# JasonTStanley/MultiDroneSim

Measured on AMD Instinct MI355X. Metric: drone-steps/sec (whole node) at N_envs×N_drones; achieved HBM GB/s vs roofline, higher is better.
Workload: dtype f32

## Files before the change

include/mds.h:

```cpp
#ifndef MDS_H
#define MDS_H

#include <stddef.h>
#include <stdint.h>

#ifdef __cplusplus
extern "C" {
#endif

#define MDS_VERSION 202
#define MDS_OBS_DIM 20
#define MDS_ACT_DIM 4
#define MDS_STATE_DIM 13
#define MDS_DES_DIM 11
#define MDS_LEM_DIM 7
#define MDS_GEO_AUX_DIM 13

typedef enum mds_status {
  MDS_OK = 0,
  MDS_EINVAL = -1,
  MDS_ENOMEM = -2,
  MDS_EHIP = -3,
  MDS_EALIGN = -4,
  MDS_ESTATE = -5,
// ... 50 lines not shown

int mds_set_origin(mds_handle* h, const double* origin_host, void* stream);

int mds_get_obs(mds_handle* h, void* obs_dev, void* stream);

int mds_step(mds_handle* h, const void* action_dev, void* obs_dev, void* stream);

int mds_set_wind(mds_handle* h, const double force_world[3]);

#define MDS_SEG_DIM 40
int mds_set_trajectory_segments(mds_handle* h, const double* segs_host, const int32_t* offsets_host,
                                const int32_t* compound_host, const double* anchor_host, int32_t total_segments, void* stream);
int mds_traj_eval(mds_handle* h, double t, void* des_dev, void* stream);

int mds_set_lemniscate(mds_handle* h, const double* params_host, void* stream);
int mds_set_geometric_gains(mds_handle* h, const mds_geometric_gains* gains);

int mds_step_geometric(mds_handle* h, double t, void* obs_dev, void* action_dev, void* stream);

int mds_rollout_geometric(mds_handle* h, double t0, int n_steps, void* obs_dev, int obs_every_step, void* stream);

int mds_rollout_step(mds_handle* h, const void* actions_dev, int n_action_sets, int first_step, int n_steps, void* obs_log_dev,
                     int log_slots, int episode_len, void* stream);
int mds_rollout_step_fused(mds_handle* h, const void* actions_dev, int n_action_sets, int first_step, int n_steps, void* obs_log_dev,
                           int log_slots, int episode_len, int steps_per_launch, void* stream);
int mds_reset_async(mds_handle* h, void* stream);

int mds_set_rollout_streams(mds_handle* h, int n_streams);
int mds_get_last_rollout_streams(const mds_handle* h);
int mds_rollout_streams_for(const mds_handle* h, int loop, int n_steps);
// ... 125 lines not shown
```

multidronesim_amd/_capi.py:

```python
from __future__ import annotations

import ctypes as C
import os

_HERE = os.path.dirname(os.path.abspath(__file__))
LIB_PATH = os.environ.get("MDS_LIB_PATH") or os.path.join(_HERE, "libmds.so")

MDS_OK = 0
MDS_F32, MDS_F64, MDS_F16, MDS_F32C = 0, 1, 2, 3
MDS_PHYSICS_DYN, MDS_PHYSICS_DYN_DRAG, MDS_PHYSICS_DYN_GND, MDS_PHYSICS_DYN_DW, MDS_PHYSICS_DYN_GND_DRAG_DW = 0, 1, 2, 3, 4
MDS_INTEGRATOR_EULER, MDS_INTEGRATOR_RK4 = 0, 1
MDS_CF2X, MDS_CF2P = 0, 1
OBS_DIM, ACT_DIM, STATE_DIM, DES_DIM, LEM_DIM, GEO_AUX_DIM, SEG_DIM = 20, 4, 13, 11, 7, 13, 40


class MdsConfig(C.Structure):
    _fields_ = [("num_envs", C.c_int32), ("num_drones", C.c_int32), ("dtype", C.c_int32), ("physics", C.c_int32),
                ("integrator", C.c_int32), ("drone_model", C.c_int32), ("pyb_freq", C.c_int32),
                ("ctrl_freq", C.c_int32), ("device", C.c_int32), ("track_last_rpm", C.c_int32),
                ("M", C.c_double), ("L", C.c_double), ("KF", C.c_double), ("KM", C.c_double), ("J", C.c_double * 3),
                ("G", C.c_double), ("thrust2weight", C.c_double), ("drag_coeff", C.c_double * 3)]


class MdsGeometricGains(C.Structure):
# ... 26 lines not shown
    "mds_last_error": (C.c_char_p, []),
    "mds_default_config": (C.c_int, [C.c_int, C.POINTER(MdsConfig)]),
    "mds_default_geometric_gains": (C.c_int, [C.POINTER(MdsGeometricGains)]),
    "mds_create": (C.c_int, [C.POINTER(MdsConfig), C.POINTER(_P)]),
    "mds_destroy": (C.c_int, [_P]),
    "mds_get_derived": (C.c_int, [_P, _PD]),
    "mds_reset": (C.c_int, [_P, _PD, _PD, _P]),
    "mds_state_ptrs": (C.c_int, [_P, C.POINTER(C.c_void_p), C.POINTER(C.c_size_t), C.POINTER(C.c_void_p)]),
    "mds_get_state": (C.c_int, [_P, _PD, _P]),
    "mds_set_state": (C.c_int, [_P, _PD, _P]),
    "mds_set_origin": (C.c_int, [_P, _PD, _P]),
    "mds_get_obs": (C.c_int, [_P, _P, _P]),
    "mds_step": (C.c_int, [_P, _P, _P, _P]),
    "mds_set_wind": (C.c_int, [_P, _PD]),
    "mds_set_lemniscate": (C.c_int, [_P, _PD, _P]),
    "mds_set_trajectory_segments": (C.c_int, [_P, _PD, C.POINTER(C.c_int32), C.POINTER(C.c_int32), _PD, C.c_int32, _P]),
    "mds_traj_eval": (C.c_int, [_P, C.c_double, _P, _P]),
    "mds_set_geometric_gains": (C.c_int, [_P, C.POINTER(MdsGeometricGains)]),
    "mds_step_geometric": (C.c_int, [_P, C.c_double, _P, _P, _P]),
    "mds_rollout_geometric": (C.c_int, [_P, C.c_double, C.c_int, _P, C.c_int, _P]),
    "mds_set_rollout_streams": (C.c_int, [_P, C.c_int]),
    "mds_get_last_rollout_streams": (C.c_int, [_P]),
    "mds_rollout_streams_for": (C.c_int, [_P, C.c_int, C.c_int]),
    "mds_set_rollout_form": (C.c_int, [_P, C.c_int, C.c_int]),
    "mds_rollout_form_for": (C.c_int, [_P, C.c_int]),
    "mds_get_last_rollout_form": (C.c_int, [_P]),
    "mds_rollout_step": (C.c_int, [_P, _P, C.c_int, C.c_int, C.c_int, _P, C.c_int, C.c_int, _P]),
    "mds_rollout_step_fused": (C.c_int, [_P, _P, C.c_int, C.c_int, C.c_int, _P, C.c_int, C.c_int, C.c_int, _P]),
    "mds_reset_async": (C.c_int, [_P, _P]),
    "mds_rollout_geometric_fused": (C.c_int, [_P, C.c_double, C.c_int, _P, _P, _P]),
# ... 98 lines not shown
```

multidronesim_amd/csrc/mds_api.hip:

```cpp
#include <hip/hip_runtime.h>
#include <math.h>
#include <stdio.h>
#include <stdlib.h>
#include <string.h>

#include <new>
#include <type_traits>
#include <unordered_map>
#include <vector>

#include "../../include/mds.h"
#include "mds_consts.hpp"
#include "mds_kernels.hip"
#include "mds_traj_image.hpp"
#ifndef MDS_PART
#define MDS_PART 3
#endif
#if MDS_PART & 2
#include "mds_cbf_kernels.hip"
#include "mds_fedce_kernels.hip"
#include "mds_fedce_omega_kernels.hip"
#include "mds_care_kernels.hip"
#else
#include "mds_cbf.hpp"
// ... 69 lines not shown
struct mds_handle {
  mds_config cfg = {};
  mds_geometric_gains gains = {};
  double wind[3] = {0.0, 0.0, 0.0};
  int n = 0;
  size_t ld = 0;
  void* state = nullptr;
  void* state_lo = nullptr;
  void* origin = nullptr;
  void* last_rpm = nullptr;
  void* lem = nullptr;
  double* scratch = nullptr;
  double* init_pose = nullptr;
  bool has_traj = false;
  int traj_mode = 0;
  double* segs = nullptr;
  int nseg_total = 0;
  int* tinfo = nullptr;
  HostParams<float> p32 = {};
  HostParams<double> p64 = {};
  bool has_cbf = false;
  mds_cbf_params cbf = {};
  int* pair_ij = nullptr;
  void* obstacles = nullptr;
  int* cbf_order = nullptr;
  int* cbf_count = nullptr;
  int cbf_calls_half[2] = {-1, -1};
  int* cbf_cost = nullptr;
  int cbf_calls = -1;
  int rollout_streams = 0;
// ... 564 lines not shown
  if (!aligned16(action) || !aligned16(obs)) return fail(MDS_EALIGN, "mds_step: action_dev/obs_dev");
  hipStream_t st = (hipStream_t)stream;
  if (h->envfx) return step_env_plain(h, action, obs, st, 0);
  launch_step_plain(h, action, obs, st);
  MDS_HIP(hipGetLastError());
  return MDS_OK;
}

int mds_set_lemniscate(mds_handle* h, const double* params, void* stream) {
  MDS_DEV(h);
  if (!h || !params) return fail(MDS_EINVAL, "mds_set_lemniscate: null argument");
  hipStream_t st = (hipStream_t)stream;
  const int n = h->n;
  double* centres = new (std::nothrow) double[(size_t)n * 3];
  if (!centres) return fail(MDS_ENOMEM, "mds_set_lemniscate: host allocation");
  for (int i = 0; i < n; ++i)
    for (int k = 0; k < 3; ++k) centres[(size_t)3 * i + k] = params[(size_t)7 * i + 2 + k];
  int rc = mds_set_origin(h, centres, stream);
  delete[] centres;
  if (rc != MDS_OK) return rc;
  MDS_HIP(hipMemcpyAsync(h->scratch, params, (size_t)n * 7 * sizeof(double), hipMemcpyHostToDevice, st));
  with_dtype(h->cfg.dtype, [&](auto DT) {
    using T = typename decltype(DT)::T;
    k_set_planes<T><<<grid_for(n, 256), 256, 0, st>>>(n, h->ld, 7, h->scratch, (T*)h->lem);
  });
  MDS_HIP(hipGetLastError());
  MDS_HIP(hipStreamSynchronize(st));
  h->has_traj = true;
  h->traj_mode = 1;
  return MDS_OK;
}

int mds_set_trajectory_segments(mds_handle* h, const double* segs, const int32_t* offsets, const int32_t* compound,
                                const double* anchor, int32_t total, void* stream) {
  MDS_DEV(h);
  if (!h || !segs || !offsets || !compound || !anchor) return fail(MDS_EINVAL, "mds_set_trajectory_segments: null argument");
  const int n = h->n;
  std::vector<int> ti;
  std::vector<double> fm;
  int nu = 0;
  const char* why = "";
  const int brc = build_traj_image(segs, offsets, compound, n, total, fm, ti, nu, &why);
  if (brc != MDS_OK) return fail(brc, why);
  int rc = mds_set_origin(h, anchor, stream);
  if (rc != MDS_OK) return rc;
  hipError_t e = hipSuccess;
  if (h->segs) (void)hipFree(h->segs);
  h->segs = nullptr;
  h->nseg_total = 0;
  if (!h->tinfo) e = hipMalloc((void**)&h->tinfo, sizeof(int) * 3 * n);
  if (e == hipSuccess) e = hipMalloc((void**)&h->segs, sizeof(double) * fm.size());
  if (e == hipSuccess) e = hipMemcpy(h->segs, fm.data(), sizeof(double) * fm.size(), hipMemcpyHostToDevice);
  if (e == hipSuccess) e = hipMemcpy(h->tinfo, ti.data(), sizeof(int) * 3 * n, hipMemcpyHostToDevice);
  if (e != hipSuccess) return fail_hip(e, "mds_set_trajectory_segments");
  h->nseg_total = nu;
  h->has_traj = true;
  h->traj_mode = 2;
  return MDS_OK;
}

int mds_traj_eval(mds_handle* h, double t, void* des, void* stream) {
  MDS_DEV(h);
  if (!h || !des) return fail(MDS_EINVAL, "mds_traj_eval: null argument");
  if (h->traj_mode == 1) return mds_lemniscate_eval(h, t, des, stream);
  if (h->traj_mode != 2) return fail(MDS_ESTATE, "mds_traj_eval: no trajectories set");
  hipStream_t st = (hipStream_t)stream;
  with_dtype(h->cfg.dtype, [&](auto DT) {
    using S = typename decltype(DT)::S;
    k_traj_eval<S><<<grid_for(h->n, 256), 256, 0, st>>>(h->n, t, SegTable{h->segs, h->nseg_total}, h->tinfo, (S*)des);
  });
  MDS_HIP(hipGetLastError());
  return MDS_OK;
// ... 18 lines not shown
  const unsigned nbatch = nb ? nb : (unsigned)((h->n + kBlock - 1) / kBlock);
  const size_t pad = nb ? split_lds_pad(h, h->traj_mode == 2 || obs) : 0;
  const dim3 grid(nbatch);
  const bool rk4 = h->cfg.integrator == MDS_INTEGRATOR_RK4, drag = has_drag(h);
  if (h->traj_mode == 2) {
    with_flags([&](auto RK4, auto DRAG) {
      with_dtype(h->cfg.dtype, [&](auto DT) {
        using T = typename decltype(DT)::T; using S = typename decltype(DT)::S;
        k_step_traj<T, S, RK4(), DRAG(), DT.COMP><<<grid, kBlock, pad, st>>>(params<T>(h).c, h->n, h->ld, t, (S*)h->state, (const T*)h->origin,
                                                                             SegTable{h->segs, h->nseg_total}, h->tinfo, (T*)rpm_track(h), (S*)obs,
                                                                             (S*)act, (int)batch0, (S*)h->state_lo);
      });
    }, rk4, drag);
    return MDS_OK;
  }
  with_flags([&](auto HAS_OBS, auto HAS_ACT, auto RK4, auto DRAG) {
    with_dtype(h->cfg.dtype, [&](auto DT) {
      using T = typename decltype(DT)::T; using S = typename decltype(DT)::S;
      k_step_geometric<T, S, HAS_OBS(), HAS_ACT(), RK4(), DRAG(), DT.COMP><<<grid, kBlock, pad, st>>>(params<T>(h).c, h->n, h->ld, t, (S*)h->state,
                                                                                                      (const T*)h->lem, (T*)rpm_track(h), (S*)obs,
                                                                                                      (S*)act, (int)batch0, (S*)h->state_lo);
    });
  }, obs != nullptr, act != nullptr, rk4, drag);
  return MDS_OK;
}

int mds_step_geometric(mds_handle* h, double t, void* obs, void* act, void* stream) {
  MDS_DEV(h);
  if (!h) return fail(MDS_EINVAL, "mds_step_geometric: null handle");
  if (!h->has_traj) return fail(MDS_ESTATE, "mds_step_geometric: call mds_set_lemniscate first");
  if (!aligned16(obs) || !aligned16(act)) return fail(MDS_EALIGN, "mds_step_geometric: obs_dev/action_dev");
  if (h->envfx) return step_env_ctrl(h, 0, t, nullptr, 0.0, obs, act, (hipStream_t)stream);
  launch_step_geometric(h, t, obs, act, (hipStream_t)stream);
  MDS_HIP(hipGetLastError());
  return MDS_OK;
}

static void launch_rollout_kernel(mds_handle* h, int ctrl, double t0, int n_steps, void* obs_log, size_t log_stride, void* obs_last, hipStream_t st) {
// ... 1 lines not shown
  const double dt = 1.0 / h->cfg.ctrl_freq;
  const int omode = obs_log == nullptr ? kObsLast : log_stride == 0 ? kObsInPlace : kObsLog;
  auto launch = [&](auto DT, auto CTRL) {
    using T = typename decltype(DT)::T; using S = typename decltype(DT)::S;
    constexpr int COMP = DT.COMP ? 1 : 0;
    const void* gain = nullptr;
    if constexpr (CTRL() >= 1) gain = h->gain_dev[CTRL() - 1];
    with_flags([&](auto RK4, auto DRAG) {
      auto roll = [&](auto OBS) {
        if (h->traj_mode == 2) {
          if constexpr (CTRL() <= 1)
            k_rollout_traj<T, S, RK4(), DRAG(), CTRL(), COMP, OBS()><<<grid, kBlock, 0, st>>>(
                params<T>(h).c, gain, h->n, h->ld, t0, dt, n_steps, (S*)h->state, (const T*)h->origin, SegTable{h->segs, h->nseg_total}, h->tinfo,
                (T*)rpm_track(h), (S*)obs_log, log_stride, (S*)obs_last, (S*)h->state_lo);
        } else {
          k_rollout_geometric<T, S, RK4(), DRAG(), CTRL(), COMP, OBS()><<<grid, kBlock, 0, st>>>(
              params<T>(h).c, gain, h->n, h->ld, t0, dt, n_steps, (S*)h->state, (const T*)h->lem, (T*)rpm_track(h), (S*)obs_log, log_stride,
              (S*)obs_last, (T*)h->ll, (const S*)obs_last, (S*)h->state_lo);
        }
      };
      constexpr bool kPerObs = sizeof(T) == 4 && !RK4() && !DRAG() && CTRL() == 0;
      if constexpr (kPerObs) with_int<kObsInPlace, kObsLog, kObsLast>(omode, roll);
      else roll(std::integral_constant<int, -1>{});
    }, h->cfg.integrator == MDS_INTEGRATOR_RK4, has_drag(h));
  };
  if (ctrl >= 2) with_int<2, 3>(ctrl, [&](auto CTRL) { with_dtype_no_half(h->cfg.dtype, [&](auto DT) { launch(DT, CTRL); }); });
  else with_int<1, 0>(ctrl, [&](auto CTRL) { with_dtype(h->cfg.dtype, [&](auto DT) { launch(DT, CTRL); }); });
}

int mds_rollout_geometric(mds_handle* h, double t0, int n_steps, void* obs, int obs_every_step, void* stream) {
  MDS_DEV(h);
  if (!h || n_steps < 0) return fail(MDS_EINVAL, "mds_rollout_geometric");
  if (!h->has_traj) return fail(MDS_ESTATE, "mds_rollout_geometric: call mds_set_lemniscate first");
// ... 1678 lines not shown
```

multidronesim_amd/csrc/mds_kernels.hip:

```cpp
#include <hip/hip_runtime.h>
#include <type_traits>

#include "mds_math.hpp"
#include "mds_traj.hpp"

namespace mds {

typedef _Float16 half_t;

constexpr int kBlock = 256;
constexpr int kWave = 64;
constexpr int kStepMinWaves = 4;

#if defined(__HIP_DEVICE_COMPILE__)
#define MDS_KEEP_V(x) asm volatile("" : "+v"(x))
#define MDS_KEEP_S(x) asm volatile("" : "+s"(x))
#else
#define MDS_KEEP_V(x) ((void)0)
#define MDS_KEEP_S(x) ((void)0)
#endif
#if defined(__HIP_DEVICE_COMPILE__) || defined(__HIPCC__)
#define MDS_CONST_AS __attribute__((address_space(4)))
#else
#define MDS_CONST_AS
// ... 421 lines not shown
  T a[4];
  load4<T, T>(lem + 4 * i, a);
  struct alignas(2 * sizeof(T)) V2 {
    T v[2];
  };
  const V2 c = *reinterpret_cast<const V2*>(lem + 4 * ld + 2 * i);
  in.P.a = a[0];
  in.P.omega = a[1];
  in.P.yaw_rate = a[2];
  in.P.phase_shift = a[3];
  in.P.cx = c.v[0];
  in.P.cy = c.v[1];
  in.P.cz = lem[6 * ld + i];
}

template <typename T, typename S, bool HAS_OBS, bool HAS_ACT, bool RK4, bool DRAG, bool COMP = false>
__device__ __forceinline__ void geo_process(const Consts<T>& c, const int n, const size_t ld, const double t, const int i,
                                            GeoIn<T>& in, S* __restrict__ state, T* __restrict__ last_rpm,
                                            S* __restrict__ obs, S* __restrict__ action_out, unsigned char* lds,
                                            S* __restrict__ state_lo = nullptr) {
  const bool valid = i < n;
  T o[kObsDim];
  if (valid) {
    State<T>& s = in.s;
    const LemniscateParams<T>& P = in.P;
    T prev[4] = {T(0), T(0), T(0), T(0)}, clipped[4], act[4];
    if (DRAG)
      for (int k = 0; k < 4; ++k) prev[k] = last_rpm[k * ld + i];
    {
      const Desired<T> des = lemniscate_local(P, t);
      const Frame<T> F = make_frame(s.q, s.w);
      T u[4];
      geometric_control<T>(c, s.p - des.p, F.R, s.v, F.av, des, u, nullptr);
      input_to_action(c, u, act);
      if (COMP) aviary_step_comp<T, RK4, DRAG>(c, s, in.r, act, prev, clipped);
      else aviary_step<T, RK4, DRAG>(c, s, F, act, prev, clipped);
    }
    if (DRAG || last_rpm)
      for (int k = 0; k < 4; ++k) last_rpm[k * ld + i] = clipped[k];
    if (HAS_ACT) store4<S, T>(action_out + (size_t)i * 4, act);
    if (HAS_OBS) pack_obs(s, V3<T>{P.cx, P.cy, P.cz}, clipped, o);
  }
  if (HAS_OBS) write_obs_rows<S, T>(lds, obs, n, i, valid, o);
  if (valid) {
    store_state<S, T>(state, ld, i, in.s);
    if (COMP) store_resid<S, T>(state_lo, ld, i, in.r);
  }
}

template <typename T, typename S, bool HAS_OBS, bool HAS_ACT, bool RK4, bool DRAG, bool COMP = false>
__global__ __launch_bounds__(kBlock, 1) void k_step_geometric(const Consts<T> c, const int n, const size_t ld, const double t,
                                                           S* __restrict__ state, const T* __restrict__ lem,
                                                           T* __restrict__ last_rpm, S* __restrict__ obs,
                                                           S* __restrict__ action_out, const int batch0,
                                                           S* __restrict__ state_lo = nullptr) {
  __shared__ __align__(16) unsigned char lds[HAS_OBS ? (kBlock * kObsDim * sizeof(S)) : 16];
  const int i = (batch0 + blockIdx.x) * kBlock + threadIdx.x;
  GeoIn<T> in;
  if (i < n) {
    load_geo_in<T, S>(state, lem, ld, i, in);
    if (COMP) load_resid<S, T>(state_lo, ld, i, in.r);
  }
  geo_process<T, S, HAS_OBS, HAS_ACT, RK4, DRAG, COMP>(c, n, ld, t, i, in, state, last_rpm, obs, action_out, lds, state_lo);
}

template <typename T, typename S, bool RK4, bool DRAG, bool COMP = false>
__global__ __launch_bounds__(kBlock) void k_step_traj(const Consts<T> c, const int n, const size_t ld, const double t,
                                                      S* __restrict__ state, const T* __restrict__ origin,
                                                      const SegTable segs, const int* __restrict__ tinfo,
                                                      T* __restrict__ last_rpm, S* __restrict__ obs, S* __restrict__ action_out,
                                                      const int batch0, S* __restrict__ state_lo = nullptr) {
  __shared__ __align__(16) unsigned char lds[kBlock * kObsDim * sizeof(S)];
  const int i = (batch0 + blockIdx.x) * kBlock + threadIdx.x;
  const bool valid = i < n;
  T o[kObsDim];
  State<T> s;
  Resid<T> r;
  if (valid) {
// ... 85 lines not shown

template <typename S>
__global__ void k_traj_eval(const int n, const double t, const SegTable segs, const int* __restrict__ tinfo,
                            S* __restrict__ des) {
  const int i = blockIdx.x * blockDim.x + threadIdx.x;
  if (i >= n) return;
  double d11[11];
  traj_eval(segs, traj_info(tinfo, i), t, d11);
  for (int k = 0; k < 11; ++k) des[(size_t)i * 11 + k] = (S)d11[k];
}

constexpr int kObsLast = 0, kObsInPlace = 1, kObsLog = 2;
template <typename T, bool RK4, bool DRAG, int CTRL, int COMP, int OBS> constexpr int rollout_min_waves() {
  return !(sizeof(T) == 4 && !RK4 && !DRAG && CTRL == 0 && COMP == 0) ? 1 : (OBS == kObsInPlace || OBS == kObsLog) ? 6 : OBS == kObsLast ? 5 : 1;
}
template <typename T, typename S, bool RK4, bool DRAG, int CTRL = 0, int COMP = -1, int OBS = -1>
__global__ __launch_bounds__(kBlock, (rollout_min_waves<T, RK4, DRAG, CTRL, COMP, OBS>())) void k_rollout_geometric(
    const Consts<T> c_arg, const void* __restrict__ Kp, const int n, const size_t ld, double t, const double ctrl_dt, const int n_steps,
    S* __restrict__ state, const T* __restrict__ lem, T* __restrict__ last_rpm, S* __restrict__ obs_log, const size_t log_stride,
    S* __restrict__ obs_last, T* __restrict__ ll = nullptr, const S* __restrict__ obs_prev = nullptr, S* __restrict__ state_lo = nullptr) {
  __shared__ __align__(16) unsigned char lds[kBlock * kObsDim * sizeof(S)];
  const bool comp = COMP < 0 ? state_lo != nullptr : COMP != 0;
  const int omode = OBS < 0 ? (obs_log == nullptr ? kObsLast : log_stride == 0 ? kObsInPlace : kObsLog) : OBS;
  constexpr bool kLean = !RK4 && COMP != 1;
  const int i = blockIdx.x * kBlock + threadIdx.x;
  const bool valid = i < n;
  if (n <= 0) return;
  const size_t il = (size_t)min(i, n - 1);
  GeoIn<T> in;
  resid_zero(in.r);
  if (comp) load_resid<S, T>(state_lo, ld, il, in.r);
  T prev[4] = {T(0), T(0), T(0), T(0)};
  T thr[4] = {T(0), T(0), T(0), T(0)};
  LowLevelState<T> L;
  L.last_omega = L.integral = {T(0), T(0), T(0)};
  load_geo_in<T, S>(state, lem, ld, il, in);
// ... 12 lines not shown
  for (int k = 0; k < n_steps; ++k) {
    T o[kObsDim];
    const bool last = k == n_steps - 1;
    const bool want = omode != kObsLast || (obs_last != nullptr && last);
#if defined(__HIP_DEVICE_COMPILE__)
    const Consts<T> MDS_CONST_AS* cp = (const Consts<T> MDS_CONST_AS*)__builtin_amdgcn_kernarg_segment_ptr();
    MDS_KEEP_S(cp);
    const Consts<T> c = kLean ? load_const(cp) : c_arg;
#else
    const Consts<T>& c = c_arg;
#endif
    T act[4], clipped[4];
    {
      if (kLean) {
        MDS_KEEP_V(in.P.a);
        MDS_KEEP_V(in.P.yaw_rate);
      }
      const Desired<T> des = lemniscate_local(in.P, t);
      T u[4];
      if (CTRL == 0) {
        if (!kCarry) {
          F = make_frame(in.s.q, in.s.w);
        } else if (kLean) {
          MDS_KEEP_V(F.r22m1);
          F.R.m[8] = T(1) + F.r22m1;
        }
        geometric_control<T>(c, in.s.p - des.p, F.R, in.s.v, F.av, des, u, nullptr);
      } else if (CTRL == 1) {
        lqr12_control<T>(c, *static_cast<const Lqr12Gain<T>*>(Kp), euler_from_quat(in.s.q), quat_rotate(in.s.q, in.s.w), in.s.v, in.s.p - des.p,
                         des.v, des.yaw, des.yaw_rate, u);
      } else if (CTRL == 2) {
        lqr_omega_control<T>(c, *static_cast<const LqrGain<T>*>(Kp), euler_from_quat(in.s.q), in.s.v, in.s.p, des.p, des.v, des.yaw, u);
      } else {
        lqr_yank_omega_control<T>(c, *static_cast<const LqrYoGain<T>*>(Kp), euler_from_quat(in.s.q), thr, in.s.v, in.s.p, des.p, des.v,
                                  des.yaw, u);
      }
      if (CTRL <= 1) input_to_action(c, u, act);
      else if (CTRL == 2) thrust_omega_control(c, (T)ctrl_dt, u, in.s.w, L, act);
      else yank_omega_control(c, (T)ctrl_dt, u, thr, in.s.w, L, act);
    }
    if (comp) aviary_step_comp<T, RK4, DRAG>(c, in.s, in.r, act, prev, clipped);
    else if (CTRL == 0) aviary_step<T, RK4, DRAG>(c, in.s, F, act, prev, clipped);
// ... 14 lines not shown
    if (omode == kObsInPlace) write_obs_rows<S, T, true, kLean>(lds, obs_log, n, i, valid, o, ro);
    else if (omode == kObsLog) write_obs_rows<S, T, false, kLean>(lds, obs_log + (size_t)k * log_stride, n, i, valid, o, ro);
    if (omode != kObsInPlace && obs_last != nullptr && last) write_obs_rows<S, T, false, kLean>(lds, obs_last, n, i, valid, o, ro);
    t = uniform_f64(t + ctrl_dt);
  }
  if (valid) {
    store_state<S, T>(state, ld, i, in.s);
    if (comp) store_resid<S, T>(state_lo, ld, i, in.r);
    if (DRAG && n_steps <= 0)
      for (int k = 0; k < 4; ++k) last_rpm[k * ld + i] = prev[k];
    if (CTRL >= 2) {
      ll[0 * ld + i] = L.last_omega.x; ll[1 * ld + i] = L.last_omega.y; ll[2 * ld + i] = L.last_omega.z;
      ll[3 * ld + i] = L.integral.x; ll[4 * ld + i] = L.integral.y; ll[5 * ld + i] = L.integral.z;
    }
  }
}

template <typename T, typename S, bool RK4, bool DRAG, int CTRL, int COMP = -1, int OBS = -1>
__global__ __launch_bounds__(kBlock) void k_rollout_traj(const Consts<T> c, const void* __restrict__ Kp, const int n, const size_t ld, double t,
                                                         const double ctrl_dt, const int n_steps, S* __restrict__ state,
                                                         const T* __restrict__ origin, const SegTable segs,
                                                         const int* __restrict__ tinfo, T* __restrict__ last_rpm,
                                                         S* __restrict__ obs_log, const size_t log_stride, S* __restrict__ obs_last,
                                                         S* __restrict__ state_lo = nullptr) {
  __shared__ __align__(16) unsigned char lds[kBlock * kObsDim * sizeof(S)];
  const bool comp = COMP < 0 ? state_lo != nullptr : COMP != 0;
  const int omode = OBS < 0 ? (obs_log == nullptr ? kObsLast : log_stride == 0 ? kObsInPlace : kObsLog) : OBS;
  const int i = blockIdx.x * kBlock + threadIdx.x;
  const bool valid = i < n;
  State<T> s;
// ... 606 lines not shown
```

multidronesim_amd/csrc/mds_math.hpp:

```cpp
#pragma once
#include <math.h>
#include <stdint.h>

#if defined(__HIPCC__)
#define MDS_HD __host__ __device__ __forceinline__
#else
#define MDS_HD inline
#endif

namespace mds {

#if defined(__HIP_DEVICE_COMPILE__)
MDS_HD float m_rcp(float x) { return __builtin_amdgcn_rcpf(x); }
MDS_HD float m_sqrt(float x) { return __builtin_amdgcn_sqrtf(x); }
MDS_HD float m_rsqrt(float x) { return __builtin_amdgcn_rsqf(x); }
#else
MDS_HD float m_rcp(float x) { return 1.0f / x; }
MDS_HD float m_sqrt(float x) { return sqrtf(x); }
MDS_HD float m_rsqrt(float x) { return 1.0f / sqrtf(x); }
#endif
MDS_HD double m_rcp(double x) { return 1.0 / x; }
MDS_HD double m_sqrt(double x) { return sqrt(x); }
MDS_HD double m_rsqrt(double x) { return 1.0 / sqrt(x); }
MDS_HD float m_fma(float a, float b, float c) { return fmaf(a, b, c); }
MDS_HD double m_fma(double a, double b, double c) { return fma(a, b, c); }
MDS_HD float m_rint(float x) { return rintf(x); }
MDS_HD double m_rint(double x) { return rint(x); }
MDS_HD float m_exp(float x) { return expf(x); }
MDS_HD double m_exp(double x) { return exp(x); }
MDS_HD float m_abs(float x) { return fabsf(x); }
MDS_HD double m_abs(double x) { return fabs(x); }
MDS_HD double m_atan2(double y, double x) { return atan2(y, x); }
MDS_HD uint64_t m_lanes(bool c) {
#if defined(__HIP_DEVICE_COMPILE__)
  return __builtin_amdgcn_ballot_w64(c);
#else
  return c;
#endif
}
MDS_HD bool m_wave_all(bool ok) { return m_lanes(!ok) == 0; }
// ... 584 lines not shown
  o[10] = s.v.x; o[11] = s.v.y; o[12] = s.v.z;
  o[13] = av.x; o[14] = av.y; o[15] = av.z;
  o[16] = rpm[0]; o[17] = rpm[1]; o[18] = rpm[2]; o[19] = rpm[3];
}
template <typename T> MDS_HD void pack_obs(const State<T>& s, V3<T> origin, const T rpm[4], T o[20]) {
  pack_obs(s, make_frame(s.q, s.w), origin, rpm, o);
}

template <typename T> struct Desired {
  V3<T> p, v, a;
  T yaw, yaw_rate;
};
template <typename T> struct LemniscateParams {
  T a, omega, cx, cy, cz, yaw_rate, phase_shift;
};
template <typename T> MDS_HD Desired<T> lemniscate_local(const LemniscateParams<T>& P, double t) {
  Desired<T> d;
  const T th = reduced_phase<T>(t, P.omega, P.phase_shift);
  T s, c;
  m_sincos(th, &s, &c);
  const T s2 = s * s, c2 = c * c;
  const T den = T(1) + s2;
  const T inv = m_rcp(den);
  const T inv2 = inv * inv;
  const T aw = P.a * P.omega;
  d.p = {P.a * s * c * inv, P.a * c * inv, T(0)};
  d.v = {-aw * (s2 * s2 + s2 + (s2 - T(1)) * c2) * inv2, -aw * s * (s2 + T(2) * c2 + T(1)) * inv2, T(0)};
  const T sin2 = T(2) * s * c, cos2 = c2 - s2, cos4 = T(1) - T(2) * sin2 * sin2;
  const T inv3 = T(-0.125) * (inv2 * inv);
  const T aw2 = aw * P.omega;
  d.a = {T(4) * aw2 * sin2 * (T(3) * cos2 + T(7)) * inv3, aw2 * c * (T(44) * cos2 + cos4 - T(21)) * inv3, T(0)};
  T sy = T(0), cy = T(1);
  if (P.yaw_rate != T(0)) {
    const T ph = reduced_phase<T>(t, P.yaw_rate, T(0));
    m_sincos(ph, &sy, &cy);
  }
  d.yaw = T(3.14159265358979323846) * sy;
  d.yaw_rate = T(3.14159265358979323846) * P.yaw_rate * cy;
  return d;
}

template <typename T> MDS_HD void input_to_action(const Consts<T>& c, const T u_in[4], T rpm[4]) {
  const T u0 = m_max(u_in[0], T(0));
  const T a = T(0.25) * u0, b1 = u_in[1] * c.inv_2L, b2 = u_in[2] * c.inv_2L, d = u_in[3] * c.inv_4r;
  T th[4] = {a - b2 - d, a + b1 + d, a + b2 - d, a - b1 + d};
  for (int i = 0; i < 4; ++i) {
// ... 3 lines not shown
}
template <typename T> MDS_HD void action_to_input(const Consts<T>& c, const T action[4], int cap_rpm, T u[4]) {
  T r[4];
  for (int i = 0; i < 4; ++i) r[i] = cap_rpm ? m_clamp(action[i], T(0), c.max_rpm) : action[i];
  u[0] = c.kf * ((r[0] * r[0] + r[1] * r[1]) + (r[2] * r[2] + r[3] * r[3]));
  u[1] = c.arm_kf * ((r[1] - r[3]) * (r[1] + r[3]));
  u[2] = c.arm_kf * ((r[2] - r[0]) * (r[2] + r[0]));
  u[3] = c.km * ((r[1] - r[0]) * (r[1] + r[0]) + (r[3] - r[2]) * (r[3] + r[2]));
}

template <typename T> struct GeoAux {
  T force;
  V3<T> w_des;
  V3<T> b1d, b2d, b3d;
};
template <typename T>
MDS_HD void geometric_control(const Consts<T>& c, V3<T> p_rel, const M3<T>& R, V3<T> v_world, V3<T> w,
                              const Desired<T>& des, T u[4], GeoAux<T>* aux) {
  const V3<T> Kp = {c.kp[0], c.kp[1], c.kp[2]}, Kv = {c.kv[0], c.kv[1], c.kv[2]};
  const V3<T> v_b = mulT(R, v_world);
  const V3<T> RTvd = mulT(R, des.v);
  const V3<T> ev = v_b - RTvd;
  V3<T> tw = des.a - hadamard(Kp, p_rel);
  tw.z += c.g_ctrl;
  const V3<T> fb_m = mulT(R, tw) - hadamard(Kv, ev) - cross(w, RTvd);
  V3<T> f_w = mul(R, c.mass * fb_m);
  T f2 = dot(f_w, f_w);
  T inv_fn = m_rsqrt(f2);
  if (f_w.z * inv_fn < c.cos_max_tilt) {
    const T scale = f_w.z * c.tan_max_tilt * m_rsqrt(m_fma(f_w.x, f_w.x, f_w.y * f_w.y));
    f_w.x *= scale;
    f_w.y *= scale;
    f2 = dot(f_w, f_w);
    inv_fn = m_rsqrt(f2);
  }
  const T fbz = dot(col(R, 2), f_w);
  T sy = T(0), cy = T(1);
  if (des.yaw != T(0)) m_sincos(des.yaw, &sy, &cy);
  const V3<T> b1c = {cy, sy, T(0)};
  const V3<T> b3d = inv_fn * f_w;
  const V3<T> c1 = cross(b3d, b1c);
  const T inv_n1 = m_rsqrt(dot(c1, c1));
  const V3<T> b2d = inv_n1 * c1;
  const V3<T> b1d = cross(b2d, b3d);
  const V3<T> b1c_dot = {-sy * des.yaw_rate, cy * des.yaw_rate, T(0)};
  const V3<T> f_dot = (c.mass * inv_fn) * mul(R, hadamard(Kp, ev));
  const V3<T> b3d_dot = reject(f_dot, b3d);
  const V3<T> inner = inv_n1 * (cross(b1c_dot, b3d) + cross(b1c, b3d_dot));
  const V3<T> b2d_dot = reject(inner, b2d);
  const V3<T> b1d_dot = cross(b3d_dot, b2d) + cross(b3d, b2d_dot);
  const V3<T> w_des = {m_fma(b1d.z, b2d_dot.x, m_fma(b2d.z, b2d_dot.y, b3d.z * b2d_dot.z)),
                       m_fma(b1d.x, b3d_dot.x, m_fma(b2d.x, b3d_dot.y, b3d.x * b3d_dot.z)),
                       m_fma(b1d.y, b1d_dot.x, m_fma(b2d.y, b1d_dot.y, b3d.y * b1d_dot.z))};
  if (aux) {
    aux->force = fbz;
    aux->w_des = w_des;
    aux->b1d = b1d;
    aux->b2d = b2d;
    aux->b3d = b3d;
  }
  const V3<T> r0 = col(R, 0), r1 = col(R, 1), r2 = col(R, 2);
  const T E12 = dot(b2d, r2) - dot(b3d, r1);
  const T E02 = dot(b1d, r2) - dot(b3d, r0);
  const T E01 = dot(b1d, r1) - dot(b2d, r0);
  const V3<T> eR = {c.kR_half[0] * E12, c.kR_half[1] * E02, c.kR_half[2] * E01};
  const V3<T> Rdw = {m_fma(b1d.x, w_des.x, m_fma(b2d.x, w_des.y, b3d.x * w_des.z)),
                     m_fma(b1d.y, w_des.x, m_fma(b2d.y, w_des.y, b3d.y * w_des.z)),
                     m_fma(b1d.z, w_des.x, m_fma(b2d.z, w_des.y, b3d.z * w_des.z))};
  const V3<T> ew = w - mulT(R, Rdw);
  const V3<T> Jw = {c.J[0] * w.x, c.J[1] * w.y, c.J[2] * w.z};
  const V3<T> wxJw = cross(w, Jw);
  u[0] = m_max(T(0), fbz);
  u[1] = c.J[0] * (-eR.x - c.kw[0] * ew.x) - wxJw.x;
  u[2] = c.J[1] * (-eR.y - c.kw[1] * ew.y) - wxJw.y;
  u[3] = c.J[2] * (-eR.z - c.kw[2] * ew.z) - wxJw.z;
}

template <typename T> struct LowLevelState {
  V3<T> last_omega, integral;
};
template <typename T>
// ... 266 lines not shown
```

multidronesim_amd/envs/BaseAviary.py:

```python
from __future__ import annotations

import ctypes as C
import time

import numpy as np
import torch

from .. import _capi as capi
from .._device import DTYPE_BY_NAME, TORCH_DTYPE, default_device_index, forget_env_device, note_env_device, require_gpu, stream_ptr, to_device
from ..utils.enums import DroneModel, Physics

__all__ = ["BaseAviary", "DroneModel", "Physics"]

_PHYSICS_MAP = {Physics.DYN: capi.MDS_PHYSICS_DYN, Physics.PYB: capi.MDS_PHYSICS_DYN,
                Physics.PYB_DRAG: capi.MDS_PHYSICS_DYN_DRAG, Physics.PYB_GND: capi.MDS_PHYSICS_DYN_GND,
                Physics.PYB_DW: capi.MDS_PHYSICS_DYN_DW, Physics.PYB_GND_DRAG_DW: capi.MDS_PHYSICS_DYN_GND_DRAG_DW}
_MODEL_MAP = {DroneModel.CF2X: capi.MDS_CF2X, DroneModel.CF2P: capi.MDS_CF2P}
_PYB_SUBSTITUTED = (Physics.PYB, Physics.PYB_DRAG, Physics.PYB_GND, Physics.PYB_DW, Physics.PYB_GND_DRAG_DW)


class BaseAviary:

    _warned_pyb = False

# ... 309 lines not shown
        self._require_open()
        capi.check(self._lib.mds_set_rollout_streams(self._h, C.c_int(int(n_streams))), "mds_set_rollout_streams")

    def last_rollout_streams(self) -> int:
        self._require_open()
        return int(self._lib.mds_get_last_rollout_streams(self._h))

    def rollout_streams_for(self, n_steps: int, cbf: bool = False) -> int:
        self._require_open()
        return int(self._lib.mds_rollout_streams_for(self._h, C.c_int(1 if cbf else 0), C.c_int(int(n_steps))))

    def set_rollout_form(self, form: int = 0, steps_per_launch: int = 0):
        self._require_open()
        capi.check(self._lib.mds_set_rollout_form(self._h, C.c_int(int(form)), C.c_int(int(steps_per_launch))), "mds_set_rollout_form")

    def rollout_form_for(self, n_steps: int) -> int:
        self._require_open()
        return int(self._lib.mds_rollout_form_for(self._h, C.c_int(int(n_steps))))

    def last_rollout_form(self) -> int:
        self._require_open()
        return int(self._lib.mds_get_last_rollout_form(self._h))

    def rollout_geometric_fused(self, t0: float, n_steps: int, log: bool = False, log_out: torch.Tensor | None = None,
                                controller: str = "geometric"):
        self._require_open()
        if log and log_out is None:
            log_out = torch.empty((n_steps, self.NUM_ENVS, self.NUM_DRONES, capi.OBS_DIM), dtype=self.dtype, device=self.device)
        fn = {"lqr": self._lib.mds_rollout_lqr_fused, "geometric": self._lib.mds_rollout_geometric_fused,
              "nominal": self._lib.mds_rollout_nominal_fused}[controller]
# ... 139 lines not shown
```

Baseline: 73.62 billion.

## Add yaw-free specialised geometric control kernels for zero-yaw lemniscate trajectories

When every lemniscate's yaw rate is zero, the host picks new Y0 kernel variants for the per-step and rollout geometric paths. These drop the yaw sincos and yaw bookkeeping, and simplify the b1c/b2d cross products knowing b1c = (1,0,0) and b2d.x = 0. This cuts ALU work per drone-step in a compute-heavy integrator kernel. It adds more template instantiations, and uses asm barriers to keep rounding close to the general path.

Measured after the change: 78.54 billion (median of 6 runs). 1.07x the previous value.

```diff
diff --git a/include/mds.h b/include/mds.h
--- a/include/mds.h
+++ b/include/mds.h
@@ -88,6 +88,8 @@
 int mds_traj_eval(mds_handle* h, double t, void* des_dev, void* stream);
 
 int mds_set_lemniscate(mds_handle* h, const double* params_host, void* stream);
+int mds_traj_yaw_free(mds_handle* h);
+int mds_set_traj_specialisation(mds_handle* h, int on);
 int mds_set_geometric_gains(mds_handle* h, const mds_geometric_gains* gains);
 
 int mds_step_geometric(mds_handle* h, double t, void* obs_dev, void* action_dev, void* stream);
diff --git a/multidronesim_amd/_capi.py b/multidronesim_amd/_capi.py
--- a/multidronesim_amd/_capi.py
+++ b/multidronesim_amd/_capi.py
@@ -64,6 +64,8 @@
     "mds_step": (C.c_int, [_P, _P, _P, _P]),
     "mds_set_wind": (C.c_int, [_P, _PD]),
     "mds_set_lemniscate": (C.c_int, [_P, _PD, _P]),
+    "mds_traj_yaw_free": (C.c_int, [_P]),
+    "mds_set_traj_specialisation": (C.c_int, [_P, C.c_int]),
     "mds_set_trajectory_segments": (C.c_int, [_P, _PD, C.POINTER(C.c_int32), C.POINTER(C.c_int32), _PD, C.c_int32, _P]),
     "mds_traj_eval": (C.c_int, [_P, C.c_double, _P, _P]),
     "mds_set_geometric_gains": (C.c_int, [_P, C.POINTER(MdsGeometricGains)]),
diff --git a/multidronesim_amd/csrc/mds_api.hip b/multidronesim_amd/csrc/mds_api.hip
--- a/multidronesim_amd/csrc/mds_api.hip
+++ b/multidronesim_amd/csrc/mds_api.hip
@@ -107,6 +107,8 @@
   double* init_pose = nullptr;
   bool has_traj = false;
   int traj_mode = 0;
+  bool traj_yaw_free = false;
+  bool traj_spec = true;
   double* segs = nullptr;
   int nseg_total = 0;
   int* tinfo = nullptr;
@@ -701,8 +703,11 @@
   const int n = h->n;
   double* centres = new (std::nothrow) double[(size_t)n * 3];
   if (!centres) return fail(MDS_ENOMEM, "mds_set_lemniscate: host allocation");
-  for (int i = 0; i < n; ++i)
+  bool yaw_free = true;
+  for (int i = 0; i < n; ++i) {
     for (int k = 0; k < 3; ++k) centres[(size_t)3 * i + k] = params[(size_t)7 * i + 2 + k];
+    yaw_free = yaw_free && params[(size_t)7 * i + 5] == 0.0;
+  }
   int rc = mds_set_origin(h, centres, stream);
   delete[] centres;
   if (rc != MDS_OK) return rc;
@@ -715,8 +720,19 @@
   MDS_HIP(hipStreamSynchronize(st));
   h->has_traj = true;
   h->traj_mode = 1;
-  return MDS_OK;
-}
+  h->traj_yaw_free = yaw_free;
+  return MDS_OK;
+}
+
+int mds_traj_yaw_free(mds_handle* h) { return h && h->traj_yaw_free ? 1 : 0; }
+
+int mds_set_traj_specialisation(mds_handle* h, int on) {
+  if (!h) return fail(MDS_EINVAL, "mds_set_traj_specialisation: null handle");
+  h->traj_spec = on != 0;
+  return MDS_OK;
+}
+
+static bool use_yaw_free(const mds_handle* h) { return h->traj_mode == 1 && h->traj_yaw_free && h->traj_spec; }
 
 int mds_set_trajectory_segments(mds_handle* h, const double* segs, const int32_t* offsets, const int32_t* compound,
                                 const double* anchor, int32_t total, void* stream) {
@@ -743,6 +759,7 @@
   h->nseg_total = nu;
   h->has_traj = true;
   h->traj_mode = 2;
+  h->traj_yaw_free = false;
   return MDS_OK;
 }
 
@@ -791,14 +808,15 @@
     }, rk4, drag);
     return MDS_OK;
   }
-  with_flags([&](auto HAS_OBS, auto HAS_ACT, auto RK4, auto DRAG) {
+  with_flags([&](auto Y0, auto HAS_OBS, auto HAS_ACT, auto RK4, auto DRAG) {
     with_dtype(h->cfg.dtype, [&](auto DT) {
       using T = typename decltype(DT)::T; using S = typename decltype(DT)::S;
-      k_step_geometric<T, S, HAS_OBS(), HAS_ACT(), RK4(), DRAG(), DT.COMP><<<grid, kBlock, pad, st>>>(params<T>(h).c, h->n, h->ld, t, (S*)h->state,
-                                                                                                      (const T*)h->lem, (T*)rpm_track(h), (S*)obs,
-                                                                                                      (S*)act, (int)batch0, (S*)h->state_lo);
+      auto* const k = Y0() ? &k_step_geometric_y0<T, S, HAS_OBS(), HAS_ACT(), RK4(), DRAG(), DT.COMP>
+                           : &k_step_geometric<T, S, HAS_OBS(), HAS_ACT(), RK4(), DRAG(), DT.COMP>;
+      k<<<grid, kBlock, pad, st>>>(params<T>(h).c, h->n, h->ld, t, (S*)h->state, (const T*)h->lem, (T*)rpm_track(h), (S*)obs, (S*)act, (int)batch0,
+                                   (S*)h->state_lo);
     });
-  }, obs != nullptr, act != nullptr, rk4, drag);
+  }, use_yaw_free(h), obs != nullptr, act != nullptr, rk4, drag);
   return MDS_OK;
 }
 
@@ -830,9 +848,11 @@
                 params<T>(h).c, gain, h->n, h->ld, t0, dt, n_steps, (S*)h->state, (const T*)h->origin, SegTable{h->segs, h->nseg_total}, h->tinfo,
                 (T*)rpm_track(h), (S*)obs_log, log_stride, (S*)obs_last, (S*)h->state_lo);
         } else {
-          k_rollout_geometric<T, S, RK4(), DRAG(), CTRL(), COMP, OBS()><<<grid, kBlock, 0, st>>>(
-              params<T>(h).c, gain, h->n, h->ld, t0, dt, n_steps, (S*)h->state, (const T*)h->lem, (T*)rpm_track(h), (S*)obs_log, log_stride,
-              (S*)obs_last, (T*)h->ll, (const S*)obs_last, (S*)h->state_lo);
+          auto* k = &k_rollout_geometric<T, S, RK4(), DRAG(), CTRL(), COMP, OBS()>;
+          if constexpr (CTRL() == 0)
+            if (use_yaw_free(h)) k = &k_rollout_geometric_y0<T, S, RK4(), DRAG(), COMP, OBS()>;
+          k<<<grid, kBlock, 0, st>>>(params<T>(h).c, gain, h->n, h->ld, t0, dt, n_steps, (S*)h->state, (const T*)h->lem, (T*)rpm_track(h), (S*)obs_log,
+                                     log_stride, (S*)obs_last, (T*)h->ll, (const S*)obs_last, (S*)h->state_lo);
         }
       };
       constexpr bool kPerObs = sizeof(T) == 4 && !RK4() && !DRAG() && CTRL() == 0;
diff --git a/multidronesim_amd/csrc/mds_kernels.hip b/multidronesim_amd/csrc/mds_kernels.hip
--- a/multidronesim_amd/csrc/mds_kernels.hip
+++ b/multidronesim_amd/csrc/mds_kernels.hip
@@ -459,7 +459,7 @@
   in.P.cz = lem[6 * ld + i];
 }
 
-template <typename T, typename S, bool HAS_OBS, bool HAS_ACT, bool RK4, bool DRAG, bool COMP = false>
+template <typename T, typename S, bool HAS_OBS, bool HAS_ACT, bool RK4, bool DRAG, bool COMP = false, bool Y0 = false>
 __device__ __forceinline__ void geo_process(const Consts<T>& c, const int n, const size_t ld, const double t, const int i,
                                             GeoIn<T>& in, S* __restrict__ state, T* __restrict__ last_rpm,
                                             S* __restrict__ obs, S* __restrict__ action_out, unsigned char* lds,
@@ -473,10 +473,10 @@
     if (DRAG)
       for (int k = 0; k < 4; ++k) prev[k] = last_rpm[k * ld + i];
     {
-      const Desired<T> des = lemniscate_local(P, t);
+      const Desired<T> des = lemniscate_local<T, Y0>(P, t);
       const Frame<T> F = make_frame(s.q, s.w);
       T u[4];
-      geometric_control<T>(c, s.p - des.p, F.R, s.v, F.av, des, u, nullptr);
+      geometric_control<T, Y0>(c, s.p - des.p, F.R, s.v, F.av, des, u, nullptr);
       input_to_action(c, u, act);
       if (COMP) aviary_step_comp<T, RK4, DRAG>(c, s, in.r, act, prev, clipped);
       else aviary_step<T, RK4, DRAG>(c, s, F, act, prev, clipped);
@@ -493,6 +493,19 @@
   }
 }
 
+template <typename T, typename S, bool HAS_OBS, bool HAS_ACT, bool RK4, bool DRAG, bool COMP, bool Y0>
+__device__ __forceinline__ void step_geometric_body(unsigned char* lds, const Consts<T>& c, const int n, const size_t ld, const double t,
+                                                    S* __restrict__ state, const T* __restrict__ lem, T* __restrict__ last_rpm,
+                                                    S* __restrict__ obs, S* __restrict__ action_out, const int batch0,
+                                                    S* __restrict__ state_lo) {
+  const int i = (batch0 + blockIdx.x) * kBlock + threadIdx.x;
+  GeoIn<T> in;
+  if (i < n) {
+    load_geo_in<T, S>(state, lem, ld, i, in);
+    if (COMP) load_resid<S, T>(state_lo, ld, i, in.r);
+  }
+  geo_process<T, S, HAS_OBS, HAS_ACT, RK4, DRAG, COMP, Y0>(c, n, ld, t, i, in, state, last_rpm, obs, action_out, lds, state_lo);
+}
 template <typename T, typename S, bool HAS_OBS, bool HAS_ACT, bool RK4, bool DRAG, bool COMP = false>
 __global__ __launch_bounds__(kBlock, 1) void k_step_geometric(const Consts<T> c, const int n, const size_t ld, const double t,
                                                            S* __restrict__ state, const T* __restrict__ lem,
@@ -500,13 +513,16 @@
                                                            S* __restrict__ action_out, const int batch0,
                                                            S* __restrict__ state_lo = nullptr) {
   __shared__ __align__(16) unsigned char lds[HAS_OBS ? (kBlock * kObsDim * sizeof(S)) : 16];
-  const int i = (batch0 + blockIdx.x) * kBlock + threadIdx.x;
-  GeoIn<T> in;
-  if (i < n) {
-    load_geo_in<T, S>(state, lem, ld, i, in);
-    if (COMP) load_resid<S, T>(state_lo, ld, i, in.r);
-  }
-  geo_process<T, S, HAS_OBS, HAS_ACT, RK4, DRAG, COMP>(c, n, ld, t, i, in, state, last_rpm, obs, action_out, lds, state_lo);
+  step_geometric_body<T, S, HAS_OBS, HAS_ACT, RK4, DRAG, COMP, false>(lds, c, n, ld, t, state, lem, last_rpm, obs, action_out, batch0, state_lo);
+}
+template <typename T, typename S, bool HAS_OBS, bool HAS_ACT, bool RK4, bool DRAG, bool COMP = false>
+__global__ __launch_bounds__(kBlock, 1) void k_step_geometric_y0(const Consts<T> c, const int n, const size_t ld, const double t,
+                                                              S* __restrict__ state, const T* __restrict__ lem,
+                                                              T* __restrict__ last_rpm, S* __restrict__ obs,
+                                                              S* __restrict__ action_out, const int batch0,
+                                                              S* __restrict__ state_lo = nullptr) {
+  __shared__ __align__(16) unsigned char lds[HAS_OBS ? (kBlock * kObsDim * sizeof(S)) : 16];
+  step_geometric_body<T, S, HAS_OBS, HAS_ACT, RK4, DRAG, COMP, true>(lds, c, n, ld, t, state, lem, last_rpm, obs, action_out, batch0, state_lo);
 }
 
 template <typename T, typename S, bool RK4, bool DRAG, bool COMP = false>
@@ -622,12 +638,12 @@
 template <typename T, bool RK4, bool DRAG, int CTRL, int COMP, int OBS> constexpr int rollout_min_waves() {
   return !(sizeof(T) == 4 && !RK4 && !DRAG && CTRL == 0 && COMP == 0) ? 1 : (OBS == kObsInPlace || OBS == kObsLog) ? 6 : OBS == kObsLast ? 5 : 1;
 }
-template <typename T, typename S, bool RK4, bool DRAG, int CTRL = 0, int COMP = -1, int OBS = -1>
-__global__ __launch_bounds__(kBlock, (rollout_min_waves<T, RK4, DRAG, CTRL, COMP, OBS>())) void k_rollout_geometric(
-    const Consts<T> c_arg, const void* __restrict__ Kp, const int n, const size_t ld, double t, const double ctrl_dt, const int n_steps,
-    S* __restrict__ state, const T* __restrict__ lem, T* __restrict__ last_rpm, S* __restrict__ obs_log, const size_t log_stride,
-    S* __restrict__ obs_last, T* __restrict__ ll = nullptr, const S* __restrict__ obs_prev = nullptr, S* __restrict__ state_lo = nullptr) {
-  __shared__ __align__(16) unsigned char lds[kBlock * kObsDim * sizeof(S)];
+template <typename T, typename S, bool RK4, bool DRAG, int CTRL, int COMP, int OBS, bool Y0>
+__device__ __forceinline__ void rollout_geometric_body(
+    unsigned char* lds, const Consts<T>& c_arg, const void* __restrict__ Kp, const int n, const size_t ld, double t, const double ctrl_dt,
+    const int n_steps, S* __restrict__ state, const T* __restrict__ lem, T* __restrict__ last_rpm, S* __restrict__ obs_log,
+    const size_t log_stride, S* __restrict__ obs_last, T* __restrict__ ll, const S* __restrict__ obs_prev, S* __restrict__ state_lo) {
+  static_assert(!Y0 || CTRL == 0, "the yaw-free form is GeometricControl's");
   const bool comp = COMP < 0 ? state_lo != nullptr : COMP != 0;
   const int omode = OBS < 0 ? (obs_log == nullptr ? kObsLast : log_stride == 0 ? kObsInPlace : kObsLog) : OBS;
   constexpr bool kLean = !RK4 && COMP != 1;
@@ -670,9 +686,9 @@
     {
       if (kLean) {
         MDS_KEEP_V(in.P.a);
-        MDS_KEEP_V(in.P.yaw_rate);
+        if (!Y0) MDS_KEEP_V(in.P.yaw_rate);
       }
-      const Desired<T> des = lemniscate_local(in.P, t);
+      const Desired<T> des = lemniscate_local<T, Y0>(in.P, t);
       T u[4];
       if (CTRL == 0) {
         if (!kCarry) {
@@ -681,7 +697,7 @@
           MDS_KEEP_V(F.r22m1);
           F.R.m[8] = T(1) + F.r22m1;
         }
-        geometric_control<T>(c, in.s.p - des.p, F.R, in.s.v, F.av, des, u, nullptr);
+        geometric_control<T, Y0>(c, in.s.p - des.p, F.R, in.s.v, F.av, des, u, nullptr);
       } else if (CTRL == 1) {
         lqr12_control<T>(c, *static_cast<const Lqr12Gain<T>*>(Kp), euler_from_quat(in.s.q), quat_rotate(in.s.q, in.s.w), in.s.v, in.s.p - des.p,
                          des.v, des.yaw, des.yaw_rate, u);
@@ -726,6 +742,24 @@
       ll[3 * ld + i] = L.integral.x; ll[4 * ld + i] = L.integral.y; ll[5 * ld + i] = L.integral.z;
     }
   }
+}
+template <typename T, typename S, bool RK4, bool DRAG, int CTRL = 0, int COMP = -1, int OBS = -1>
+__global__ __launch_bounds__(kBlock, (rollout_min_waves<T, RK4, DRAG, CTRL, COMP, OBS>())) void k_rollout_geometric(
+    const Consts<T> c_arg, const void* __restrict__ Kp, const int n, const size_t ld, double t, const double ctrl_dt, const int n_steps,
+    S* __restrict__ state, const T* __restrict__ lem, T* __restrict__ last_rpm, S* __restrict__ obs_log, const size_t log_stride,
+    S* __restrict__ obs_last, T* __restrict__ ll = nullptr, const S* __restrict__ obs_prev = nullptr, S* __restrict__ state_lo = nullptr) {
+  __shared__ __align__(16) unsigned char lds[kBlock * kObsDim * sizeof(S)];
+  rollout_geometric_body<T, S, RK4, DRAG, CTRL, COMP, OBS, false>(lds, c_arg, Kp, n, ld, t, ctrl_dt, n_steps, state, lem, last_rpm, obs_log,
+                                                                  log_stride, obs_last, ll, obs_prev, state_lo);
+}
+template <typename T, typename S, bool RK4, bool DRAG, int COMP = -1, int OBS = -1>
+__global__ __launch_bounds__(kBlock, (rollout_min_waves<T, RK4, DRAG, 0, COMP, OBS>())) void k_rollout_geometric_y0(
+    const Consts<T> c_arg, const void* __restrict__ Kp, const int n, const size_t ld, double t, const double ctrl_dt, const int n_steps,
+    S* __restrict__ state, const T* __restrict__ lem, T* __restrict__ last_rpm, S* __restrict__ obs_log, const size_t log_stride,
+    S* __restrict__ obs_last, T* __restrict__ ll = nullptr, const S* __restrict__ obs_prev = nullptr, S* __restrict__ state_lo = nullptr) {
+  __shared__ __align__(16) unsigned char lds[kBlock * kObsDim * sizeof(S)];
+  rollout_geometric_body<T, S, RK4, DRAG, 0, COMP, OBS, true>(lds, c_arg, Kp, n, ld, t, ctrl_dt, n_steps, state, lem, last_rpm, obs_log,
+                                                              log_stride, obs_last, ll, obs_prev, state_lo);
 }
 
 template <typename T, typename S, bool RK4, bool DRAG, int CTRL, int COMP = -1, int OBS = -1>
diff --git a/multidronesim_amd/csrc/mds_math.hpp b/multidronesim_amd/csrc/mds_math.hpp
--- a/multidronesim_amd/csrc/mds_math.hpp
+++ b/multidronesim_amd/csrc/mds_math.hpp
@@ -24,6 +24,15 @@
 MDS_HD double m_rsqrt(double x) { return 1.0 / sqrt(x); }
 MDS_HD float m_fma(float a, float b, float c) { return fmaf(a, b, c); }
 MDS_HD double m_fma(double a, double b, double c) { return fma(a, b, c); }
+template <typename T> MDS_HD T m_mul_rn(T a, T b) {
+  T r = a * b;
+#if defined(__HIP_DEVICE_COMPILE__)
+  asm("" : "+v"(r));
+#else
+  asm("" : "+m"(r));
+#endif
+  return r;
+}
 MDS_HD float m_rint(float x) { return rintf(x); }
 MDS_HD double m_rint(double x) { return rint(x); }
 MDS_HD float m_exp(float x) { return expf(x); }
@@ -638,7 +647,7 @@
 template <typename T> struct LemniscateParams {
   T a, omega, cx, cy, cz, yaw_rate, phase_shift;
 };
-template <typename T> MDS_HD Desired<T> lemniscate_local(const LemniscateParams<T>& P, double t) {
+template <typename T, bool Y0 = false> MDS_HD Desired<T> lemniscate_local(const LemniscateParams<T>& P, double t) {
   Desired<T> d;
   const T th = reduced_phase<T>(t, P.omega, P.phase_shift);
   T s, c;
@@ -654,6 +663,10 @@
   const T inv3 = T(-0.125) * (inv2 * inv);
   const T aw2 = aw * P.omega;
   d.a = {T(4) * aw2 * sin2 * (T(3) * cos2 + T(7)) * inv3, aw2 * c * (T(44) * cos2 + cos4 - T(21)) * inv3, T(0)};
+  if (Y0) {
+    d.yaw = d.yaw_rate = T(0);
+    return d;
+  }
   T sy = T(0), cy = T(1);
   if (P.yaw_rate != T(0)) {
     const T ph = reduced_phase<T>(t, P.yaw_rate, T(0));
@@ -687,15 +700,24 @@
   V3<T> w_des;
   V3<T> b1d, b2d, b3d;
 };
-template <typename T>
+template <typename T, bool Y0 = false>
 MDS_HD void geometric_control(const Consts<T>& c, V3<T> p_rel, const M3<T>& R, V3<T> v_world, V3<T> w,
                               const Desired<T>& des, T u[4], GeoAux<T>* aux) {
   const V3<T> Kp = {c.kp[0], c.kp[1], c.kp[2]}, Kv = {c.kv[0], c.kv[1], c.kv[2]};
   const V3<T> v_b = mulT(R, v_world);
-  const V3<T> RTvd = mulT(R, des.v);
+  V3<T> RTvd, tw;
+  if (Y0) {
+    RTvd = {m_fma(R.m[0], des.v.x, R.m[3] * des.v.y), m_fma(R.m[1], des.v.x, R.m[4] * des.v.y), m_fma(R.m[2], des.v.x, R.m[5] * des.v.y)};
+  } else {
+    RTvd = mulT(R, des.v);
+  }
   const V3<T> ev = v_b - RTvd;
-  V3<T> tw = des.a - hadamard(Kp, p_rel);
-  tw.z += c.g_ctrl;
+  if (Y0) {
+    tw = {des.a.x - Kp.x * p_rel.x, des.a.y - Kp.y * p_rel.y, c.g_ctrl - m_mul_rn(Kp.z, p_rel.z)};
+  } else {
+    tw = des.a - hadamard(Kp, p_rel);
+    tw.z += c.g_ctrl;
+  }
   const V3<T> fb_m = mulT(R, tw) - hadamard(Kv, ev) - cross(w, RTvd);
   V3<T> f_w = mul(R, c.mass * fb_m);
   T f2 = dot(f_w, f_w);
@@ -708,23 +730,40 @@
     inv_fn = m_rsqrt(f2);
   }
   const T fbz = dot(col(R, 2), f_w);
-  T sy = T(0), cy = T(1);
-  if (des.yaw != T(0)) m_sincos(des.yaw, &sy, &cy);
-  const V3<T> b1c = {cy, sy, T(0)};
   const V3<T> b3d = inv_fn * f_w;
-  const V3<T> c1 = cross(b3d, b1c);
-  const T inv_n1 = m_rsqrt(dot(c1, c1));
-  const V3<T> b2d = inv_n1 * c1;
-  const V3<T> b1d = cross(b2d, b3d);
-  const V3<T> b1c_dot = {-sy * des.yaw_rate, cy * des.yaw_rate, T(0)};
-  const V3<T> f_dot = (c.mass * inv_fn) * mul(R, hadamard(Kp, ev));
-  const V3<T> b3d_dot = reject(f_dot, b3d);
-  const V3<T> inner = inv_n1 * (cross(b1c_dot, b3d) + cross(b1c, b3d_dot));
-  const V3<T> b2d_dot = reject(inner, b2d);
-  const V3<T> b1d_dot = cross(b3d_dot, b2d) + cross(b3d, b2d_dot);
-  const V3<T> w_des = {m_fma(b1d.z, b2d_dot.x, m_fma(b2d.z, b2d_dot.y, b3d.z * b2d_dot.z)),
-                       m_fma(b1d.x, b3d_dot.x, m_fma(b2d.x, b3d_dot.y, b3d.x * b3d_dot.z)),
-                       m_fma(b1d.y, b1d_dot.x, m_fma(b2d.y, b1d_dot.y, b3d.y * b1d_dot.z))};
+  V3<T> b1d, b2d, w_des;
+  if (Y0) {
+    const T inv_n1 = m_rsqrt(m_fma(b3d.z, b3d.z, b3d.y * b3d.y));
+    b2d = {T(0), inv_n1 * b3d.z, inv_n1 * -b3d.y};
+    b1d = {m_fma(b2d.y, b3d.z, -(b2d.z * b3d.y)), b2d.z * b3d.x, -(b2d.y * b3d.x)};
+    const V3<T> f_dot = (c.mass * inv_fn) * mul(R, hadamard(Kp, ev));
+    const V3<T> b3d_dot = reject(f_dot, b3d);
+    const T inner_y = inv_n1 * -b3d_dot.z, inner_z = inv_n1 * b3d_dot.y;
+    const T d = -m_fma(b2d.y, inner_y, b2d.z * inner_z);
+    const T b2d_dot_y = m_fma(d, b2d.y, inner_y), b2d_dot_z = m_fma(d, b2d.z, inner_z);
+    const V3<T> b1d_dot = {m_fma(b3d_dot.y, b2d.z, -(b3d_dot.z * b2d.y)) + m_fma(b3d.y, b2d_dot_z, -(b3d.z * b2d_dot_y)),
+                           -m_mul_rn(b3d_dot.x, b2d.z) - m_mul_rn(b3d.x, b2d_dot_z),
+                           m_mul_rn(b3d_dot.x, b2d.y) + m_mul_rn(b3d.x, b2d_dot_y)};
+    w_des = {m_fma(b2d.z, b2d_dot_y, b3d.z * b2d_dot_z), m_fma(b1d.x, b3d_dot.x, b3d.x * b3d_dot.z),
+             m_fma(b1d.y, b1d_dot.x, m_fma(b2d.y, b1d_dot.y, b3d.y * b1d_dot.z))};
+  } else {
+    T sy = T(0), cy = T(1);
+    if (des.yaw != T(0)) m_sincos(des.yaw, &sy, &cy);
+    const V3<T> b1c = {cy, sy, T(0)};
+    const V3<T> c1 = cross(b3d, b1c);
+    const T inv_n1 = m_rsqrt(dot(c1, c1));
+    b2d = inv_n1 * c1;
+    b1d = cross(b2d, b3d);
+    const V3<T> b1c_dot = {-sy * des.yaw_rate, cy * des.yaw_rate, T(0)};
+    const V3<T> f_dot = (c.mass * inv_fn) * mul(R, hadamard(Kp, ev));
+    const V3<T> b3d_dot = reject(f_dot, b3d);
+    const V3<T> inner = inv_n1 * (cross(b1c_dot, b3d) + cross(b1c, b3d_dot));
+    const V3<T> b2d_dot = reject(inner, b2d);
+    const V3<T> b1d_dot = cross(b3d_dot, b2d) + cross(b3d, b2d_dot);
+    w_des = {m_fma(b1d.z, b2d_dot.x, m_fma(b2d.z, b2d_dot.y, b3d.z * b2d_dot.z)),
+             m_fma(b1d.x, b3d_dot.x, m_fma(b2d.x, b3d_dot.y, b3d.x * b3d_dot.z)),
+             m_fma(b1d.y, b1d_dot.x, m_fma(b2d.y, b1d_dot.y, b3d.y * b1d_dot.z))};
+  }
   if (aux) {
     aux->force = fbz;
     aux->w_des = w_des;
@@ -733,11 +772,11 @@
     aux->b3d = b3d;
   }
   const V3<T> r0 = col(R, 0), r1 = col(R, 1), r2 = col(R, 2);
-  const T E12 = dot(b2d, r2) - dot(b3d, r1);
+  const T E12 = (Y0 ? m_fma(b2d.y, r2.y, b2d.z * r2.z) : dot(b2d, r2)) - dot(b3d, r1);
   const T E02 = dot(b1d, r2) - dot(b3d, r0);
-  const T E01 = dot(b1d, r1) - dot(b2d, r0);
+  const T E01 = dot(b1d, r1) - (Y0 ? m_fma(b2d.y, r0.y, b2d.z * r0.z) : dot(b2d, r0));
   const V3<T> eR = {c.kR_half[0] * E12, c.kR_half[1] * E02, c.kR_half[2] * E01};
-  const V3<T> Rdw = {m_fma(b1d.x, w_des.x, m_fma(b2d.x, w_des.y, b3d.x * w_des.z)),
+  const V3<T> Rdw = {Y0 ? m_fma(b1d.x, w_des.x, b3d.x * w_des.z) : m_fma(b1d.x, w_des.x, m_fma(b2d.x, w_des.y, b3d.x * w_des.z)),
                      m_fma(b1d.y, w_des.x, m_fma(b2d.y, w_des.y, b3d.y * w_des.z)),
                      m_fma(b1d.z, w_des.x, m_fma(b2d.z, w_des.y, b3d.z * w_des.z))};
   const V3<T> ew = w - mulT(R, Rdw);
diff --git a/multidronesim_amd/envs/BaseAviary.py b/multidronesim_amd/envs/BaseAviary.py
--- a/multidronesim_amd/envs/BaseAviary.py
+++ b/multidronesim_amd/envs/BaseAviary.py
@@ -347,6 +347,14 @@
         self._require_open()
         capi.check(self._lib.mds_set_rollout_form(self._h, C.c_int(int(form)), C.c_int(int(steps_per_launch))), "mds_set_rollout_form")
 
+    def traj_yaw_free(self) -> bool:
+        self._require_open()
+        return bool(self._lib.mds_traj_yaw_free(self._h))
+
+    def set_traj_specialisation(self, on: bool = True):
+        self._require_open()
+        capi.check(self._lib.mds_set_traj_specialisation(self._h, C.c_int(1 if on else 0)), "mds_set_traj_specialisation")
+
     def rollout_form_for(self, n_steps: int) -> int:
         self._require_open()
         return int(self._lib.mds_rollout_form_for(self._h, C.c_int(int(n_steps))))
```
